# wangchou/whisper.coreml

Hardware: AMD Instinct MI355X
Metric: xRT (audio-s/s) large-v3 beam=5 @1/2/4/8 GPU; p50 per-token decode ms (higher is better)
Workload: dtype fp16; 1 GPU; large-v3 beam=5 transcribe() of one 600 s file, 30 s clip grid, condition_on_previous_text=False, temperature=0; model=large-v3, global_batch=20, seq_len=448

## Files before the change

### profiles/chain_trace.py

```python
import ctypes
import os
import sys

import numpy as np

REPO = os.path.dirname(os.path.dirname(os.path.abspath(__file__)))
sys.path[:0] = [os.path.join(REPO, "whisper.coreml_amd"), REPO]
import whisper
from whisper import synthetic as S
from whisper.decoding import DecodingTask

W = int(sys.argv[1]) if len(sys.argv) > 1 else 20
REPS = int(sys.argv[2]) if len(sys.argv) > 2 else 10
ADVANCE = int(sys.argv[3]) if len(sys.argv) > 3 else 0
model_name = os.environ.get("CT_MODEL", "large-v3")
dims = S.MODEL_DIMS[model_name]
m = whisper.Whisper(whisper.ModelDimensions(**dims), model_name, device=0, dtype="fp16", max_windows=W, max_group=5)
m.load_state_dict(S.synthetic_state_dict(dims, 0))
m.ctx.log_mel(S.synthetic_audio(30.0 * W, seed=1000), dims["n_mels"], padding=whisper.audio.N_SAMPLES)
m.ctx.encode([3000 * i for i in range(W)], [3000] * W)
task = DecodingTask(m, whisper.DecodingOptions(language="en", beam_size=5))
lib = m.ctx.lib
UNITS = ["proj", "kernels", "gemm", "decode"]
for u in UNITS:
    getattr(lib, f"wh_tune_ct_trace_{u}").argtypes = [ctypes.c_void_p]
    getattr(lib, f"wh_tune_ct_trace_{u}").restype = ctypes.c_int
    getattr(lib, f"wh_tune_ct_clear_{u}").restype = ctypes.c_int
SLOT_UNIT = {0: "proj", 1: "proj", 2: "proj", 3: "proj", 4: "kernels", 5: "kernels", 6: "kernels", 7: "kernels",
             8: "gemm", 9: "decode", 10: "decode", 11: "decode"}
ORDER = [(0, "qkv k_proj", ("X staged", "MFMA done")), (6, "self-attn (+qkv reduce)", None),
         (7, "cross-attn k_xattn_seg", None), (1, "cross-out k_proj", ("X staged", "MFMA done")),
         (2, "fc1 k_proj", ("X staged", "MFMA done")), (5, "reduce+GELU", None),
         (3, "fc2 k_proj", ("X staged", "MFMA done")), (4, "resid+LN (final)", ("loads landed", None)),
         (8, "vocab k_vocab_2p / k_vocab1", ("epilogue start", "half 1 staged")), (9, "selection k_logit_part", ("row combine", "window merge")),
         (10, "  merge_window (in it)", ("staged", "ranked")),
         (11, "  selection slices (marks)", ("loads", "top-k"))]

m.ctx.decode_begin(task.wh_opts(), [task.initial_tokens] * W, [task.sot_index] * W)
m.ctx.time_stage(0, 2 + ADVANCE)
rows = {s: [] for s, _, _ in ORDER}
steps = []
for rep in range(REPS):
    for u in UNITS:
        assert getattr(lib, f"wh_tune_ct_clear_{u}")() == 0
    steps.append(m.ctx.time_stage(0, 1))
    tr = {}
    for u in UNITS:
        buf = np.zeros((12, 2048, 4), dtype=np.uint64)
        assert getattr(lib, f"wh_tune_ct_trace_{u}")(buf.ctypes.data) == 0
        tr[u] = buf.astype(np.int64)
    base = None
    for slot, name, phases in ORDER:
        t = tr[SLOT_UNIT[slot]][slot]
        t = t[t[:, 0] > 0]
        if len(t) == 0:
            continue
        if base is None:
            base = t[:, 0].min()
        rel = (t - base) * 0.01
        ends = rel[:, 3][t[:, 3] > 0]
        rows[slot].append(dict(n=len(t), s0=rel[:, 0].min(), s1=rel[:, 0].max(),
                               p1=np.median(rel[:, 1][t[:, 1] > 0]) if (t[:, 1] > 0).any() else np.nan,
                               p2=np.median(rel[:, 2][t[:, 2] > 0]) if (t[:, 2] > 0).any() else np.nan,
                               e_med=np.median(ends) if len(ends) else np.nan, e1=ends.max() if len(ends) else np.nan,
                               p1max=rel[:, 1][t[:, 1] > 0].max() if (t[:, 1] > 0).any() else np.nan,
                               p2max=rel[:, 2][t[:, 2] > 0].max() if (t[:, 2] > 0).any() else np.nan))
print(f"{model_name} fp16, {W} windows x beam 5 ({5 * W} rows), after {2 + ADVANCE} steps: "
      f"step graph {np.median(steps):.3f} ms "
      f"(median of {REPS}); times in us from layer 31's qkv first workgroup start, medians over {REPS} steps")
print(f"{'launch':28s} {'WGs':>5s} {'gap':>6s} {'start0':>7s} {'startN':>7s} {'phase1':>7s} {'phase2':>7s} "
      f"{'end med':>7s} {'end max':>7s} {'span':>6s}")
prev_end = None
for slot, name, phases in ORDER:
    if not rows[slot]:
        continue
    agg = {k: float(np.nanmedian([r[k] for r in rows[slot]])) for k in rows[slot][0]}
    gap = agg["s0"] - prev_end if prev_end is not None else float("nan")
    print(f"{name:28s} {int(agg['n']):5d} {gap:6.2f} {agg['s0']:7.2f} {agg['s1']:7.2f} {agg['p1']:7.2f} "
          f"{agg['p2']:7.2f} {agg['e_med']:7.2f} {agg['e1']:7.2f} {agg['e1'] - agg['s0']:6.2f}"
          f"   (phase maxima {agg['p1max']:.2f} / {agg['p2max']:.2f})")
    prev_end = agg["e1"]
```

### whisper.coreml_amd/csrc/wh_kernels.hip

```cpp
#include "wh_kernels.h"

#include <cstdio>
#include <type_traits>
#include <cstdlib>

namespace wh {

template <typename T>
__global__ __launch_bounds__(256) void k_layernorm(const float* __restrict__ x, T* __restrict__ y, const float* __restrict__ gamma,
                                                   const float* __restrict__ beta, int rows, int n, float eps,
                                                   const int* __restrict__ rows_in) {
  const int row = blockIdx.x * 4 + (threadIdx.x >> 6);
  const int lane = threadIdx.x & 63;
  if (row >= rows) return;
  const int src = rows_in ? rows_in[row] : row;
  const float* xr = x + (int64_t)src * n;
  constexpr int MAXV = 8;
  float4_t v[MAXV];
  const int nv = n >> 2;
#pragma unroll
  for (int i = 0; i < MAXV; ++i) {
    const int c = lane + 64 * i;
    if (c < nv) v[i] = load4f(xr + 4 * c);
  }
// ... 400 lines not shown
      CT_END(CT_SELF_ATTN);
      return;
    }
  }
  if constexpr (sizeof(T) == 2) {
    int sv[8];
#pragma unroll
    for (int i = 0; i < 8; ++i) sv[i] = an[min(lane + 64 * i, ctx - 1)];
    qs[lane] = to_f32(q_lane);
#pragma unroll
    for (int i = 0; i < 8; ++i) {
      const int pp = lane + 64 * i;
      if (pp <= pos) slot_of[pp] = (pp == pos ? sl : sv[i]) * slotB;
    }
    asm volatile("s_waitcnt lgkmcnt(0)" ::: "memory");
    const int kg = lane >> 3, dc = (lane & 7) * 8;
    float m = -INFINITY, lsum = 0.f, o[8];
#pragma unroll
    for (int e = 0; e < 8; ++e) o[e] = 0.f;
    for (int p0 = 0; p0 <= pos; p0 += 128) {
      const int pa = min(p0 + lane, pos), pb = min(p0 + 64 + lane, pos);
      const int ra = baseB + slot_of[pa] + pa * ROWB, rb = baseB + slot_of[pb] + pb * ROWB;
      Frag<T> ka[8], kb[8], vf[16];
#pragma unroll
      for (int c = 0; c < 8; ++c) frag_load_buf(ka[c], rk, ra + 8 * c * TB);
#pragma unroll
      for (int c = 0; c < 8; ++c) frag_load_buf(kb[c], rk, rb + 8 * c * TB);
#pragma unroll
      for (int u = 0; u < 16; ++u) {
        const int pc = min(p0 + kg + 8 * u, pos);
        frag_load_buf(vf[u], rv, baseB + slot_of[pc] + pc * ROWB + dc * TB);
      }
      __builtin_amdgcn_sched_barrier(0);
      float sa = 0.f, sb = 0.f;
#pragma unroll
      for (int c = 0; c < 8; ++c) {
        const float4_t q0 = *reinterpret_cast<const float4_t*>(&qs[8 * c]);
        const float4_t q1 = *reinterpret_cast<const float4_t*>(&qs[8 * c + 4]);
#pragma unroll
        for (int e = 0; e < 8; ++e) {
          const float qe = e < 4 ? q0[e] : q1[e - 4];
          sa += qe * to_f32(ka[c].v[e]);
          sb += qe * to_f32(kb[c].v[e]);
        }
      }
      const bool va = p0 + lane <= pos, vb = p0 + 64 + lane <= pos;
      const float mp = wave_max(fmaxf(va ? sa : -INFINITY, vb ? sb : -INFINITY));
      const float mn = fmaxf(m, mp), scale = __expf(m - mn);
      m = mn;
      const float ea = va ? __expf(sa - m) : 0.f, eb = vb ? __expf(sb - m) : 0.f;
      lsum = lsum * scale + wave_sum(ea + eb);
      sc[lane] = ea;
      sc[64 + lane] = eb;
      asm volatile("s_waitcnt lgkmcnt(0)" ::: "memory");
#pragma unroll
      for (int e = 0; e < 8; ++e) o[e] *= scale;
#pragma unroll
      for (int u = 0; u < 16; ++u) {
        const float pw = sc[kg + 8 * u];
#pragma unroll
        for (int e = 0; e < 8; ++e) o[e] += pw * to_f32(vf[u].v[e]);
      }
    }
#pragma unroll
    for (int e = 0; e < 8; ++e) {
      o[e] = xor8_sum(o[e]);
      o[e] = xor16_sum(o[e]);
      o[e] = xor32_sum(o[e]);
    }
    if (kg == 0) {
      const float inv = 1.f / lsum;
      T* op = out + (int64_t)row * ldo + h * 64 + dc;
      store4(op, o[0] * inv, o[1] * inv, o[2] * inv, o[3] * inv);
      store4(op + 4, o[4] * inv, o[5] * inv, o[6] * inv, o[7] * inv);
    }
    CT_END(CT_SELF_ATTN);
    return;
  }
  qs[lane] = to_f32(q_lane);
  asm volatile("s_waitcnt lgkmcnt(0)" ::: "memory");
  unpack_q();
  float mx = -INFINITY;
  for (int p = lane; p <= pos; p += 64) {
    const int slot = ((p == pos) ? sl : an[p]) * slotB;
    slot_of[p] = slot;
    const int kr = baseB + slot + p * ROWB;
    float s = 0.f;
#pragma unroll
    for (int c = 0; c < 64; c += 8) {
      Frag<T> f;
      frag_load_buf(f, rk, kr + c * TB);
#pragma unroll
      for (int e = 0; e < 8; ++e) s += qv[c + e] * to_f32(f.v[e]);
    }
    sc[p] = s;
    mx = fmaxf(mx, s);
  }
  mx = wave_max(mx);
  float sum = 0.f;
  for (int p = lane; p <= pos; p += 64) {
    const float e = __expf(sc[p] - mx);
    sc[p] = e;
    sum += e;
  }
  sum = wave_sum(sum);
  __syncthreads();
  const int kg = lane >> 3, dc = (lane & 7) * 8;
  float o[8];
#pragma unroll
  for (int e = 0; e < 8; ++e) o[e] = 0.f;
  int p = kg;
  for (; p + 24 <= pos; p += 32) {
    Frag<T> f[4];
#pragma unroll
    for (int u = 0; u < 4; ++u) frag_load_buf(f[u], rv, baseB + slot_of[p + 8 * u] + (p + 8 * u) * ROWB + dc * TB);
#pragma unroll
    for (int u = 0; u < 4; ++u) {
      const float pw = sc[p + 8 * u];
#pragma unroll
      for (int e = 0; e < 8; ++e) o[e] += pw * to_f32(f[u].v[e]);
    }
  }
  for (; p <= pos; p += 8) {
    Frag<T> f;
    frag_load_buf(f, rv, baseB + slot_of[p] + p * ROWB + dc * TB);
    const float pw = sc[p];
#pragma unroll
    for (int e = 0; e < 8; ++e) o[e] += pw * to_f32(f.v[e]);
  }
#pragma unroll
  for (int e = 0; e < 8; ++e) {
    o[e] = xor8_sum(o[e]);
    o[e] = xor16_sum(o[e]);
    o[e] = xor32_sum(o[e]);
  }
  if (kg == 0) {
    const float inv = 1.f / sum;
    T* op = out + (int64_t)row * ldo + h * 64 + dc;
    store4(op, o[0] * inv, o[1] * inv, o[2] * inv, o[3] * inv);
    store4(op + 4, o[4] * inv, o[5] * inv, o[6] * inv, o[7] * inv);
  }
  CT_END(CT_SELF_ATTN);
}

template <typename T>
void launch_self_attn(const T* q, int ldq, const T* kc, const T* vc, const int* rw, const int* rs, const int* rp,
                      const int* anc, int anc_beams, int nbeam, int H, int ctx, T* out, int ldo, int rows,
                      hipStream_t st) {
  if (rows <= 0) return;
  k_self_attn<T><<<dim3(rows, H), 64, 0, st>>>(q, ldq, kc, vc, rw, rs, rp, anc, anc_beams, nbeam, H, ctx, out, ldo,
                                               self_attn_kco_min()), wh_launched("k_self_attn");
}

template <typename T, typename S = float>
__global__ __launch_bounds__(64) __attribute__((amdgpu_waves_per_eu(1, 2))) void k_self_attn_qkv(const S* __restrict__ part, int nsplit, int64_t part_stride,
                                                      const float* __restrict__ bqkv, int ns, T* __restrict__ kc,
                                                      T* __restrict__ vc, const int* __restrict__ row_win,
                                                      const int* __restrict__ row_slot, const int* __restrict__ row_pos,
                                                      const int* __restrict__ anc, int anc_beams, int nbeam, int H,
                                                      int ctx, T* __restrict__ out, int ldo, int kco_min = 0) {
  __shared__ float sc[512];
  __shared__ int slot_of[512];
  __shared__ float qs[64], vs[64];
  const int lane = threadIdx.x, G = anc_beams;
  CT_MARK(CT_SELF_ATTN, 0);
  const int L = xcd_remap(blockIdx.x, gridDim.x), sl = L % G, wh = L / G, h = wh % H, w = wh / H, row = w * G + sl;
  const int* an = anc + ((int64_t)w * anc_beams + sl) * ctx;
  const int64_t head_stride = (int64_t)ctx * 64;
  const int64_t wbase = (int64_t)w * nbeam;
  auto kv_off = [&](int slot, int p) -> int64_t { return ((wbase + slot) * H + h) * head_stride + (int64_t)p * 64; };
  constexpr int TB = (int)sizeof(T), ROWB = 64 * TB;
  const int slotB = H * ctx * ROWB, baseB = ((int)wbase * H + h) * ctx * ROWB;
  const auto rk = wt_rsrc(kc), rv = wt_rsrc(vc);
  const int pos = row_pos[row];
  int sv[8];
#pragma unroll
  for (int i = 0; i < 8; ++i) sv[i] = an[min(lane + 64 * i, ctx - 1)];
  float qd, kd, vd;
  {
    constexpr bool H16 = sizeof(S) == 2;
    const S* pr = part + (int64_t)row * 3 * ns + h * 64 + lane;
    qd = bqkv[h * 64 + lane];
    kd = bqkv[ns + h * 64 + lane];
    vd = bqkv[2 * ns + h * 64 + lane];
    S a0[16], a1[16], a2[16];
#pragma unroll
    for (int z = 0; z < 16; ++z)
      if (H16 || z < nsplit) {
        const int64_t zo = (int64_t)(H16 ? min(z, nsplit - 1) : z) * part_stride;
        a0[z] = pr[zo];
        a1[z] = pr[zo + ns];
        a2[z] = pr[zo + 2 * ns];
      }
    if constexpr (H16) {
      asm volatile("" ::"s"(pos));
#pragma unroll
      for (int z = 0; z < 16; ++z) asm volatile("" ::"v"(a0[z]), "v"(a1[z]), "v"(a2[z]));
    }
    auto f32 = [](S r) -> float { return (float)r; };
#pragma unroll
    for (int z = 0; z < 16; ++z)
      if (z < nsplit) {
        qd += f32(a0[z]);
        kd += f32(a1[z]);
        vd += f32(a2[z]);
      }
  }
  for (int i = 0; i < 8; ++i)
    if (lane + 64 * i < pos) slot_of[lane + 64 * i] = sv[i] * slotB;
  const int plast = max(pos - 1, 0);
  const T qT = from_f32<T>(qd), kT = from_f32<T>(kd), vT = from_f32<T>(vd);
  kc[kv_off(sl, pos) + lane] = kT;
  vc[kv_off(sl, pos) + lane] = vT;
  qs[lane] = to_f32(qT);
  vs[lane] = to_f32(vT);
  const float s_cur = wave_sum(to_f32(qT) * to_f32(kT));
  asm volatile("s_waitcnt lgkmcnt(0)" ::: "memory");
  if constexpr (sizeof(T) == 2) {
    const int kg = lane >> 3, dc = (lane & 7) * 8;
    float m = s_cur, lsum = 0.f, o[8];
#pragma unroll
    for (int e = 0; e < 8; ++e) o[e] = 0.f;
    float qd8[8];
#pragma unroll
    for (int e = 0; e < 8; ++e) qd8[e] = qs[dc + e];
    auto load = [&](auto kc, int p0, Frag<T>(&k)[8], Frag<T>(&v)[8]) {
      if constexpr (decltype(kc)::value) {
        int off[8];
#pragma unroll
        for (int u = 0; u < 8; ++u) {
          const int pc = min(p0 + kg + 8 * u, plast);
          off[u] = baseB + slot_of[pc] + pc * ROWB + dc * TB;
        }
#pragma unroll
        for (int u = 0; u < 8; ++u) frag_load_buf(k[u], rk, off[u]);
#pragma unroll
        for (int u = 0; u < 8; ++u) frag_load_buf(v[u], rv, off[u]);
        return;
      }
      const int pa = min(p0 + lane, plast);
      const int ra = baseB + slot_of[pa] + pa * ROWB;
#pragma unroll
      for (int c = 0; c < 8; ++c) frag_load_buf(k[c], rk, ra + 8 * c * TB);
#pragma unroll
      for (int u = 0; u < 8; ++u) {
        const int pc = min(p0 + kg + 8 * u, plast);
        frag_load_buf(v[u], rv, baseB + slot_of[pc] + pc * ROWB + dc * TB);
      }
    };
    auto pass = [&](auto kc, int p0, const Frag<T>(&k)[8], const Frag<T>(&v)[8]) {
      if constexpr (decltype(kc)::value) {
        kco_pass<T, 8>(qd8, k, v, p0 + kg, pos, m, lsum, o);
        return;
      }
      float sa = 0.f;
#pragma unroll
      for (int c = 0; c < 8; ++c) {
        const float4_t q0 = *reinterpret_cast<const float4_t*>(&qs[8 * c]);
        const float4_t q1 = *reinterpret_cast<const float4_t*>(&qs[8 * c + 4]);
#pragma unroll
        for (int e = 0; e < 8; ++e) sa += (e < 4 ? q0[e] : q1[e - 4]) * to_f32(k[c].v[e]);
      }
      const bool va = p0 + lane < pos;
      const float mp = wave_max(va ? sa : -INFINITY);
      const float mn = fmaxf(m, mp), scale = __expf(m - mn);
      m = mn;
      const float ea = va ? __expf(sa - m) : 0.f;
      lsum = lsum * scale + wave_sum(ea);
      sc[lane] = ea;
      asm volatile("s_waitcnt lgkmcnt(0)" ::: "memory");
#pragma unroll
      for (int e = 0; e < 8; ++e) o[e] *= scale;
#pragma unroll
      for (int u = 0; u < 8; ++u) {
        const float pw = sc[kg + 8 * u];
#pragma unroll
        for (int e = 0; e < 8; ++e) o[e] += pw * to_f32(v[u].v[e]);
      }
    };
    auto run = [&](auto kc) {
      Frag<T> ka[8], va[8], kb[8], vb[8];
      if (pos > 0) load(kc, 0, ka, va);
      int p0 = 0;
      for (; p0 + 64 < pos; p0 += 128) {
        load(kc, p0 + 64, kb, vb);
        pass(kc, p0, ka, va);
        if (p0 + 128 < pos) load(kc, p0 + 128, ka, va);
        pass(kc, p0 + 64, kb, vb);
      }
      if (p0 < pos) pass(kc, p0, ka, va);
    };
    if (pos > kco_min) run(std::true_type());
    else run(std::false_type());
#pragma unroll
    for (int e = 0; e < 8; ++e) {
      o[e] = xor8_sum(o[e]);
      o[e] = xor16_sum(o[e]);
      o[e] = xor32_sum(o[e]);
    }
    if (kg == 0) {
      const float e_cur = __expf(s_cur - m), inv = 1.f / (lsum + e_cur);
#pragma unroll
      for (int e = 0; e < 8; ++e) o[e] = (o[e] + e_cur * vs[dc + e]) * inv;
      T* op = out + (int64_t)row * ldo + h * 64 + dc;
      store4(op, o[0], o[1], o[2], o[3]);
      store4(op + 4, o[4], o[5], o[6], o[7]);
    }
    CT_END(CT_SELF_ATTN);
    return;
  }
  float qv[64];
#pragma unroll
  for (int c = 0; c < 64; ++c) qv[c] = qs[c];
  float mx = s_cur;
  for (int p0 = 0; p0 < pos; p0 += 128) {
    const int pa = min(p0 + lane, plast), pb = min(p0 + 64 + lane, plast);
    const int ra = baseB + slot_of[pa] + pa * ROWB, rb = baseB + slot_of[pb] + pb * ROWB;
    Frag<T> ka[8], kb[8];
#pragma unroll
    for (int c = 0; c < 8; ++c) frag_load_buf(ka[c], rk, ra + 8 * c * TB);
#pragma unroll
    for (int c = 0; c < 8; ++c) frag_load_buf(kb[c], rk, rb + 8 * c * TB);
    __builtin_amdgcn_sched_barrier(0);
    float sa = 0.f, sb = 0.f;
#pragma unroll
    for (int c = 0; c < 8; ++c)
#pragma unroll
      for (int e = 0; e < 8; ++e) {
        sa += qv[8 * c + e] * to_f32(ka[c].v[e]);
        sb += qv[8 * c + e] * to_f32(kb[c].v[e]);
      }
    if (p0 + lane < pos) {
      sc[p0 + lane] = sa;
      mx = fmaxf(mx, sa);
    }
    if (p0 + 64 + lane < pos) {
      sc[p0 + 64 + lane] = sb;
      mx = fmaxf(mx, sb);
    }
  }
  mx = wave_max(mx);
  float sum = 0.f;
  for (int p = lane; p < pos; p += 64) {
    const float e = __expf(sc[p] - mx);
    sc[p] = e;
    sum += e;
  }
  const float e_cur = __expf(s_cur - mx);
  sum = wave_sum(sum) + e_cur;
  asm volatile("s_waitcnt lgkmcnt(0)" ::: "memory");
  const int kg = lane >> 3, dc = (lane & 7) * 8;
  float o[8];
#pragma unroll
  for (int e = 0; e < 8; ++e) o[e] = 0.f;
  for (int p0 = kg; p0 < pos; p0 += 64) {
    Frag<T> f[8];
    float pw[8];
#pragma unroll
    for (int u = 0; u < 8; ++u) {
      const int pc = min(p0 + 8 * u, plast);
      frag_load_buf(f[u], rv, baseB + slot_of[pc] + pc * ROWB + dc * TB);
      pw[u] = p0 + 8 * u < pos ? sc[pc] : 0.f;
    }
    __builtin_amdgcn_sched_barrier(0);
#pragma unroll
    for (int u = 0; u < 8; ++u)
#pragma unroll
      for (int e = 0; e < 8; ++e) o[e] += pw[u] * to_f32(f[u].v[e]);
  }
#pragma unroll
  for (int e = 0; e < 8; ++e) {
    o[e] = xor8_sum(o[e]);
    o[e] = xor16_sum(o[e]);
    o[e] = xor32_sum(o[e]);
  }
  if (kg == 0) {
    const float inv = 1.f / sum;
#pragma unroll
    for (int e = 0; e < 8; ++e) o[e] = (o[e] + e_cur * vs[dc + e]) * inv;
    T* op = out + (int64_t)row * ldo + h * 64 + dc;
    store4(op, o[0], o[1], o[2], o[3]);
    store4(op + 4, o[4], o[5], o[6], o[7]);
  }
  CT_END(CT_SELF_ATTN);
}

int self_attn_kco_min() {
  static const int v = [] {
    const char* e = tune_env("WHISPER_HIP_SA_KCO_MIN");
    return e ? atoi(e) : 64;
  }();
  return v;
}
template <typename T>
int launch_self_attn_qkv(const float* part, int nsplit, int64_t part_stride, const float* bqkv, int ns, T* kc, T* vc,
                          const int* rw, const int* rs, const int* rp, const int* anc, int anc_beams, int nbeam, int H,
                          int ctx, T* out, int ldo, int rows, hipStream_t st, int slab_half) {
  if (rows <= 0) return 0;
  if (anc_beams < 1 || rows % anc_beams || nsplit > 16) return -1;
  if (slab_half) {
    if constexpr (sizeof(T) == 2) {
      k_self_attn_qkv<T, half_t><<<rows * H, 64, 0, st>>>(reinterpret_cast<const half_t*>(part), nsplit, part_stride,
                                                         bqkv, ns, kc, vc, rw, rs, rp, anc, anc_beams, nbeam, H, ctx,
                                                         out, ldo, self_attn_kco_min()), wh_launched("k_self_attn_qkv");
      return 0;
    }
    return -1;
  }
  k_self_attn_qkv<T><<<rows * H, 64, 0, st>>>(part, nsplit, part_stride, bqkv, ns, kc, vc, rw, rs, rp, anc, anc_beams,
                                             nbeam, H, ctx, out, ldo, self_attn_kco_min()), wh_launched("k_self_attn_qkv");
  return 0;
}

template <typename T, int ACT, typename S = float>
__global__ __launch_bounds__(256) void k_reduce_store(const S* __restrict__ part, int nsplit, int64_t part_stride,
                                                      const float* __restrict__ bias, T* __restrict__ out, int ldo, int M,
                                                      int N) {
  const int i = (int)(blockIdx.x * 256 + threadIdx.x) * 4;
  CT_MARK(CT_REDUCE, 0);
  if (i >= M * N) return;
  const int m = (int)((unsigned)i / (unsigned)N), n = i - m * N;
  typedef typename std::conditional<sizeof(S) == 2, half4_t, float4_t>::type R4;
  R4 pp[16];
#pragma unroll
  for (int z = 0; z < 16; ++z)
    if (z < nsplit) pp[z] = *reinterpret_cast<const R4*>(part + z * part_stride + i);
  float4_t v = bias ? load4f(bias + n) : (float4_t){0.f, 0.f, 0.f, 0.f};
#pragma unroll
  for (int z = 0; z < 16; ++z)
    if (z < nsplit) v += (float4_t){(float)pp[z][0], (float)pp[z][1], (float)pp[z][2], (float)pp[z][3]};
  if (ACT) {
#pragma unroll
    for (int j = 0; j < 4; ++j) v[j] = gelu_f(v[j]);
  }
  store4(out + (int64_t)m * ldo + n, v[0], v[1], v[2], v[3]);
  CT_END(CT_REDUCE);
}

template <typename T>
void launch_reduce_store(const float* part, int nsplit, int64_t part_stride, const float* bias, T* out, int ldo, int M,
                         int N, int gelu, hipStream_t st, int slab_half) {
  if (M <= 0) return;
  if ((int64_t)M * N >= (int64_t)1 << 31) {
    wh_set_launch_error("launch_reduce_store: M x N >= 2^31");
    return;
  }
  const int64_t tot = (int64_t)M * N / 4;
  const unsigned nb = (unsigned)((tot + 255) / 256);
  if (slab_half) {
    if constexpr (sizeof(T) == 2) {
      const half_t* ph = reinterpret_cast<const half_t*>(part);
      if (gelu) k_reduce_store<T, 1, half_t><<<nb, 256, 0, st>>>(ph, nsplit, part_stride, bias, out, ldo, M, N), wh_launched("k_reduce_store");
      else k_reduce_store<T, 0, half_t><<<nb, 256, 0, st>>>(ph, nsplit, part_stride, bias, out, ldo, M, N), wh_launched("k_reduce_store");
    } else {
      wh_set_launch_error("launch_reduce_store: fp16 slabs in an fp32 context");
    }
    return;
  }
  if (gelu) k_reduce_store<T, 1><<<nb, 256, 0, st>>>(part, nsplit, part_stride, bias, out, ldo, M, N), wh_launched("k_reduce_store");
  else k_reduce_store<T, 0><<<nb, 256, 0, st>>>(part, nsplit, part_stride, bias, out, ldo, M, N), wh_launched("k_reduce_store");
}

template <typename T, int NW, int QZ>
__global__ __launch_bounds__(64 * NW) void k_cross_attn(const T* __restrict__ q, int ldq, const T* ck,
                                                    const T* cvt, int Tk, int H, int nsplit,
                                                    const int* __restrict__ win_row0, const int* __restrict__ win_nrows,
                                                    const int* __restrict__ win_slot, int64_t win_stride,
                                                    float* __restrict__ po, float* __restrict__ pm, float* __restrict__ pl,
                                                    float* qk_out, const int* qk_map, int qk_rows, XQPart xq) {
  __shared__ float red_m[NW][16], red_l[NW][16];
  __shared__ float red_o[NW][64][17];
  constexpr bool QP = QZ > 0;
  __shared__ __attribute__((aligned(16))) T qs[QP ? 32 : 1][72];
  const int wi = blockIdx.x, h = blockIdx.y, sp = blockIdx.z;
  const int tid = threadIdx.x, lane = tid & 63, wave = tid >> 6;
  const int r = lane & 15, g = lane >> 4;
  const int row0 = win_row0[wi], nrows = win_nrows[wi];
  const int kt0 = (sp * NW + wave) * 64;
  const bool active = kt0 < Tk;
  const int qslot = qk_map ? qk_map[h] : -1;
  const T* kbase = ck + (int64_t)win_slot[wi] * win_stride + (int64_t)h * TKP * 64;
  const T* vbase = cvt + (int64_t)win_slot[wi] * win_stride + (int64_t)h * 64 * TKP;
  constexpr float LOG2E = 1.4426950408889634f;
  const int ktl = active ? kt0 : 0;
  Frag<T> kf[4][2], vf[4][2];
#pragma unroll
  for (int kt = 0; kt < 4; ++kt) {
    const T* kp = kbase + (int64_t)(ktl + kt * 16 + r) * 64 + 8 * g;
    frag_load(kf[kt][0], kp);
    frag_load(kf[kt][1], kp + 32);
  }
  float4_t qv = (float4_t){0.f, 0.f, 0.f, 0.f}, pp[QP ? QZ : 1];
  __builtin_amdgcn_sched_barrier(0);
  if constexpr (QP) {
    const int t = tid & 255, qq = min(t >> 4, nrows - 1), c = h * 64 + (t & 15) * 4;
    const float* src = xq.part + (int64_t)(row0 + qq) * ldq + c;
#pragma unroll
    for (int z = 0; z < QZ; ++z) pp[z] = load4f(src + z * xq.stride);
    qv = load4f(xq.bias + c);
  }
  __builtin_amdgcn_sched_barrier(0);
#pragma unroll
  for (int dt = 0; dt < 4; ++dt)
#pragma unroll
    for (int s = 0; s < 2; ++s) frag_load(vf[dt][s], vbase + ((int64_t)(ktl >> 6) * 64 + dt * 16 + r) * 64 + 32 * s + 8 * g);
  if constexpr (QP) {
#pragma unroll
    for (int z = 0; z < QZ; ++z) qv += pp[z];
    store4(&qs[tid >> 4][(tid & 15) * 4], qv[0], qv[1], qv[2], qv[3]);
    asm volatile("s_waitcnt lgkmcnt(0)\n\ts_barrier" ::: "memory");
  }
  for (int rt = 0; rt < nrows; rt += 16) {
    int qr = rt + r;
    const bool qvalid = qr < nrows;
    if (!qvalid) qr = nrows - 1;
    float m = -INFINITY, l = 0.f;
    float4_t acc[4];
#pragma unroll
    for (int i = 0; i < 4; ++i) acc[i] = (float4_t){0.f, 0.f, 0.f, 0.f};
    if (active) {
      Frag<T> qf[2];
      if constexpr (QP) {
        frag_load(qf[0], &qs[qr][8 * g]);
        frag_load(qf[1], &qs[qr][32 + 8 * g]);
      } else {
        const T* qp = q + (int64_t)(row0 + qr) * ldq + h * 64 + 8 * g;
        frag_load(qf[0], qp);
        frag_load(qf[1], qp + 32);
      }
      float4_t sc[4];
#pragma unroll
      for (int kt = 0; kt < 4; ++kt) {
        sc[kt] = (float4_t){0.f, 0.f, 0.f, 0.f};
        mfma_step(sc[kt], kf[kt][0], qf[0]);
        mfma_step(sc[kt], kf[kt][1], qf[1]);
      }
      float mx = -INFINITY;
#pragma unroll
      for (int kt = 0; kt < 4; ++kt)
#pragma unroll
        for (int j = 0; j < 4; ++j) {
          const int key = kt0 + kt * 16 + 4 * g + j;
          if (key >= Tk) sc[kt][j] = -INFINITY;
          else if (qslot >= 0 && qvalid) qk_out[((int64_t)qslot * qk_rows + row0 + qr) * Tk + key] = sc[kt][j];
          mx = fmaxf(mx, sc[kt][j]);
        }
      mx = xor16_max(mx);
      mx = xor32_max(mx);
      m = mx;
      Frag<T> pf[2];
      float ps = 0.f;
#pragma unroll
      for (int kt = 0; kt < 4; ++kt)
#pragma unroll
        for (int j = 0; j < 4; ++j) {
          const float p = hw_exp2((sc[kt][j] - m) * LOG2E);
          ps += p;
// ... 832 lines not shown
```

### whisper.coreml_amd/csrc/wh_runtime.hip

```cpp
#include <hip/hip_runtime.h>

#include <algorithm>
#include <chrono>
#include <cmath>
#include <cstdio>
#include <cstring>
#include <set>
#include <string>
#include <vector>

#include "whisper_hip.h"
#include "wh_align.h"
#include "wh_audio.h"
#include "wh_gemm.h"
#include "wh_host.h"
#include "wh_kernels.h"

using namespace wh;

static thread_local std::string g_release_error;

namespace {

constexpr int CTX = 448;
// ... 606 lines not shown
    g.out_f32 = part; g.ldo = N; g.ksplit = *ks;
    return gemm(X, ldx, W, nullptr, R, N, K, EPI_PARTIAL, g);
  }

  int resid(const T* X, int K, const T* W, const float* b, int R, const float* lg, const float* lb) {
    const int n = ns;
    GemmArgs g;
    if (R > 128) {
      g.out_f32 = x_d; g.ldo = n;
      TRY(gemm(X, K, W, b, R, n, K, EPI_RESID, g));
      launch_resid_ln<T>(x_d, nullptr, 0, 0, nullptr, xn_d, lg, lb, R, n, 1e-5f, st);
    } else {
      int ks = 0;
      TRY(partial(X, K, W, R, n, K, &ks));
      launch_resid_ln<T>(x_d, part, ks, (int64_t)R * n, b, xn_d, lg, lb, R, n, 1e-5f, st, slab_h);
    }
    return 0;
  }
  int proj(const T* W, const float* b, int R, int N, T* out, int gelu, bool skinny) {
    GemmArgs g;
    if (skinny) {
      int ks = 0;
      TRY(partial(xn_d, ns, W, R, N, ns, &ks));
      launch_reduce_store<T>(part, ks, (int64_t)R * N, b, out, N, R, N, gelu, st, slab_h);
    } else {
      g.out = out; g.ldo = N;
      TRY(gemm(xn_d, ns, W, b, R, N, ns, gelu ? EPI_STORE_GELU : EPI_STORE, g));
    }
    return 0;
  }

  int sa_probe_ks = 1;
  int sa_probe_half = 0;
  int dec_layers(int R, const int* rw, const int* rs, const int* rp, int ancG, int nwin, const int* wr0, const int* wnr,
                 const int* wsl, float* aqk, const int* qkmap, int qkrows, bool step = false,
                 const int* anc = nullptr) {
    const int* A = anc ? anc : S.anc;
    const int n = ns;
    const bool skinny = step && R <= 128;
    GemmArgs g;
    final_x = nullptr;
    if (step && !qkmap && p1_active(R, nwin))
      return dec_layers_p1(R, rw, rs, rp, ancG, nwin, wr0, wnr, wsl, A);
    launch_layernorm<T>(x_d, xn_d, dec[0].ln1_g, dec[0].ln1_b, R, n, 1e-5f, nullptr, st);
    for (int l = 0; l < Ld; ++l) {
      auto& e = dec[l];
      if (skinny) {
        int ks = 0;
        TRY(partial(xn_d, n, e.wqkv, R, 3 * n, n, &ks, slab16_qkv()));
        sa_probe_ks = ks;
        sa_probe_half = slab_h;
        if (launch_self_attn_qkv<T>(part, ks, (int64_t)R * 3 * n, e.bqkv, n, kc[l], vc[l], rw, rs, rp, A, ancG,
                                    Gcap, nh, CTX, att_d, n, R, st, slab_h))
          return fail(-20, "self-attention rows are not a whole number of beam groups");
      } else {
        g = GemmArgs();
        g.out = q_d; g.ldo = n; g.hs_state = n; g.hs_heads = nh;
        g.row_win = rw; g.row_slot = rs; g.row_pos = rp; g.kc = kc[l]; g.vc = vc[l]; g.kv_beams = Gcap; g.kv_ctx = CTX;
        TRY(gemm(xn_d, n, e.wqkv, e.bqkv, R, 3 * n, n, EPI_QKV_DEC, g));
        launch_self_attn<T>(q_d, n, kc[l], vc[l], rw, rs, rp, A, ancG, Gcap, nh, CTX, att_d, n, R, st);
      }
      TRY(resid(att_d, n, e.wo, e.bo, R, e.lnx_g, e.lnx_b));
      XQPart xq;
      if (skinny) xq = step_xq(ancG);
      if (skinny && xq_proj_active(ancG)) {
        xq.qx = xn_d; xq.qwf = e.wqx_f; xq.bias = e.bqx;
      } else if (skinny && xq_fused) {
        int ks = 0;
        TRY(partial(xn_d, n, e.wqx, R, n, n, &ks));
        if (cross_attn_q_slabs(ks)) {
          xq.part = part; xq.part_half = slab_h; xq.stride = (int64_t)R * n; xq.z = ks; xq.bias = e.bqx;
        } else {
          launch_reduce_store<T>(part, ks, (int64_t)R * n, e.bqx, q_d, n, R, n, 0, st, slab_h);
        }
      } else {
        TRY(proj(e.wqx, e.bqx, R, n, q_d, 0, skinny));
      }
      const T* ck = ckv + (size_t)(2 * l) * Wcap * TKP * n;
      const T* cv = ckv + (size_t)(2 * l + 1) * Wcap * TKP * n;
      launch_cross_attn<T>(q_d, n, ck, cv, 1500, nh, NSPLIT, nwin, wr0, wnr, wsl, (int64_t)TKP * n, po, pm, pl, att_d,
                           n, R, aqk, qkmap ? qkmap + l * nh : nullptr, qkrows, st, xq);
      TRY(resid(att_d, n, e.wox, e.box, R, e.ln2_g, e.ln2_b));
      TRY(proj(e.w1, e.b1, R, 4 * n, hm_d, 1, skinny));
      const bool last = l + 1 == Ld;
      TRY(resid(hm_d, 4 * n, e.w2, e.b2, R, last ? ln_g : dec[l + 1].ln1_g, last ? ln_b : dec[l + 1].ln1_b));
    }
    return 0;
  }

  static bool p1_enabled() {
    static const bool on = [] {
      const char* e = tune_env("WHISPER_HIP_P1");
      return !(e && e[0] == '0');
    }();
    return on;
  }

  int p1(GemmArgs& g, int epi, bool ln) {
    g.p1_slab = p1_slab;
    g.p1_cnt = p1_cnt;
    g.p1_slabs = P1_SLABS;
    const bool tev = proj_ev_n < (int)proj_ev.size() / 2;
    const int rc = tev ? launch_proj1<T>(g, epi, ln, st, proj_ev[2 * proj_ev_n], proj_ev[2 * proj_ev_n + 1])
                       : launch_proj1<T>(g, epi, ln, st);
    if (tev && rc == 0) ++proj_ev_n;
    return rc == 0 ? 0 : fail(-20, "k_proj1 launch failed code " + std::to_string(rc));
  }

  int layer_projections(int l, int R) {
    const int n = ns;
    auto& e = dec[l];
    if (p1_active(R, cur_nwin)) {
      GemmArgs g;
      g.W = e.wqkv; g.bias = e.bqkv; g.M = R; g.N = 3 * n; g.K = n;
      g.xf32 = x_d; g.ln_g = e.ln1_g; g.ln_b = e.ln1_b; g.ln_eps = 1e-5f;
      g.out = q_d; g.ldo = n; g.hs_state = n; g.hs_heads = nh;
      g.row_win = st_row_win; g.row_slot = st_row_slot; g.row_pos = row_pos; g.kc = kc[l]; g.vc = vc[l];
      g.kv_beams = Gcap; g.kv_ctx = CTX;
      TRY(p1(g, EPI_QKV_DEC, true));
      struct Q { const T* X; int K; const T* W; const float* b; int N; int epi; const float* lg; const float* lb; T* out; };
      const Q qs[5] = {{att_d, n, e.wo, e.bo, n, EPI_RESID, nullptr, nullptr, nullptr},
                       {nullptr, n, e.wqx, e.bqx, n, EPI_STORE, e.lnx_g, e.lnx_b, q_d},
                       {att_d, n, e.wox, e.box, n, EPI_RESID, nullptr, nullptr, nullptr},
                       {nullptr, n, e.w1, e.b1, 4 * n, EPI_STORE_GELU, e.ln2_g, e.ln2_b, hm_d},
                       {hm_d, 4 * n, e.w2, e.b2, n, EPI_RESID, nullptr, nullptr, nullptr}};
      for (const Q& q : qs) {
        g = GemmArgs();
        g.W = q.W; g.bias = q.b; g.M = R; g.N = q.N; g.K = q.K;
        if (q.lg) {
          g.xf32 = x_d; g.ln_g = q.lg; g.ln_b = q.lb; g.ln_eps = 1e-5f; g.out = q.out; g.ldo = q.N;
        } else {
          g.X = q.X; g.ldx = q.K; g.out_f32 = x_d; g.ldo = n;
        }
        TRY(p1(g, q.epi, q.lg != nullptr));
      }
      return 0;
    }
    struct P { const T* X; int K; const T* W; int N; } ps[6] = {
        {xn_d, n, e.wqkv, 3 * n}, {att_d, n, e.wo, n}, {xn_d, n, e.wqx, n},
        {att_d, n, e.wox, n},     {xn_d, n, e.w1, 4 * n}, {hm_d, 4 * n, e.w2, n}};
    for (auto& p : ps) {
      if (p.W == e.wqx && xq_proj_active(cur_G)) continue;
      int ks = 0;
      TRY(partial(p.X, p.K, p.W, R, p.N, p.K, &ks));
    }
    return 0;
  }

  bool p1_active(int R, int n_win) const { return n_win == 1 && p1_enabled() && proj1_supported(R, ns); }
  std::string step_kernels(int n_win, int group) const override {
    const bool p1 = p1_active(n_win * group, n_win), h = sizeof(T) == 2;
    return std::string("proj=") + (p1 ? "k_proj1" : "k_proj") + ",xattn=k_xattn_seg" +
           (!p1 && xq_proj_active(group) ? "<qproj>" : "") + ",self_attn=" +
           (p1 ? (h ? "k_self_attn<kco>" : "k_self_attn") : h ? "k_self_attn_qkv<pipe+kco>" : "k_self_attn_qkv") +
           ",tail=vocab+k_logit_part";
  }

  int dec_layers_p1(int R, const int* rw, const int* rs, const int* rp, int ancG, int nwin, const int* wr0,
                    const int* wnr, const int* wsl, const int* A) {
    const int n = ns;
    float* xc = x_d;
    float* xo = x2_d;
    const float* pend = nullptr;
    auto ln_in = [&](GemmArgs& g, const float* lg, const float* lb) {
      g.xf32 = xc; g.ln_g = lg; g.ln_b = lb; g.ln_eps = 1e-5f;
      if (pend) { g.res_slab = p1_slab; g.res_bias = pend; g.x_out = xo; }
    };
    auto ln_done = [&]() {
      if (pend) { std::swap(xc, xo); pend = nullptr; }
    };
    auto resid = [&](const T* X, int K, const T* W, const float* b, bool defer) -> int {
      GemmArgs g;
      g.X = X; g.ldx = K; g.W = W; g.bias = b; g.M = R; g.N = n; g.K = K; g.out_f32 = xc; g.ldo = n;
      g.p1_defer = defer;
      TRY(p1(g, EPI_RESID, false));
      if (defer) pend = b;
      return 0;
    };
    for (int l = 0; l < Ld; ++l) {
      auto& e = dec[l];
      GemmArgs g;
      g.W = e.wqkv; g.bias = e.bqkv; g.M = R; g.N = 3 * n; g.K = n;
      ln_in(g, e.ln1_g, e.ln1_b);
      g.out = q_d; g.ldo = n; g.hs_state = n; g.hs_heads = nh;
      g.row_win = rw; g.row_slot = rs; g.row_pos = rp; g.kc = kc[l]; g.vc = vc[l]; g.kv_beams = Gcap; g.kv_ctx = CTX;
      TRY(p1(g, EPI_QKV_DEC, true));
      ln_done();
      launch_self_attn<T>(q_d, n, kc[l], vc[l], rw, rs, rp, A, ancG, Gcap, nh, CTX, att_d, n, R, st);
      TRY(resid(att_d, n, e.wo, e.bo, false));
      XQPart xq = step_xq(ancG);
      g = GemmArgs();
      g.W = e.wqx; g.bias = e.bqx; g.M = R; g.N = n; g.K = n;
      ln_in(g, e.lnx_g, e.lnx_b);
      g.out = q_d; g.ldo = n;
      TRY(p1(g, EPI_STORE, true));
      ln_done();
      const T* ck = ckv + (size_t)(2 * l) * Wcap * TKP * n;
      const T* cv = ckv + (size_t)(2 * l + 1) * Wcap * TKP * n;
      launch_cross_attn<T>(q_d, n, ck, cv, 1500, nh, NSPLIT, nwin, wr0, wnr, wsl, (int64_t)TKP * n, po, pm, pl, att_d,
                           n, R, nullptr, nullptr, 0, st, xq);
      TRY(resid(att_d, n, e.wox, e.box, false));
      g = GemmArgs();
      g.W = e.w1; g.bias = e.b1; g.M = R; g.N = 4 * n; g.K = n;
      ln_in(g, e.ln2_g, e.ln2_b);
      g.out = hm_d; g.ldo = 4 * n;
      TRY(p1(g, EPI_STORE_GELU, true));
      ln_done();
      TRY(resid(hm_d, 4 * n, e.w2, e.b2, l + 1 < Ld));
    }
    final_x = xc;
    return 0;
  }

  const float* final_x = nullptr;
  int vocab(const int* rows_sel, int R, float* out) {
    GemmArgs g;
    g.out_f32 = out; g.ldo = V; g.x_rows = rows_sel;
    if (final_x && rows_sel) return fail(-20, "vocab: a row gather after the k_proj1 layers (xn_d not written)");
    if (final_x) {
      g.xf32 = final_x; g.ln_g = ln_g; g.ln_b = ln_b; g.ln_eps = 1e-5f;
    }
    return gemm(xn_d, ns, E, nullptr, R, V, ns, EPI_F32_COLS, g);
  }

  int set_opts(const wh_decode_opts* o, int n_win) {
    if (o->group < 1 || o->group > Gcap) return fail(-11, "group exceeds context max_group");
    const int mc = !o->beam ? 0
                   : o->max_candidates > 0 ? o->max_candidates
                                           : (int)std::nearbyint((double)o->group * (o->patience > 0 ? o->patience : 1.0));
    if (o->beam && (mc < 1 || mc > 16)) return fail(-11, "max_candidates out of range (1..16)");
    if (o->no_repeat_ngram < 0 || o->no_repeat_ngram > 16)
      return fail(-11, "no_repeat_ngram " + std::to_string(o->no_repeat_ngram) + " out of range (0..16)");
    if (!(o->repetition_penalty >= 0.f) || std::isinf(o->repetition_penalty))
      return fail(-11, "repetition_penalty must be finite and not negative (0 or 1: off)");
    const float pen = o->repetition_penalty == 0.f ? 1.f : o->repetition_penalty;
    const bool rep_on = o->no_repeat_ngram > 0 || pen != 1.f;
    if (rep_on || !bias_tab.empty()) {
      DecOpts q = DecOpts();
      q.V = V; q.ts_begin = o->timestamp_begin;
      if (!logit_slices(S, q, n_win))
        return fail(-11, std::string(!rep_on ? "phrase_bias" : bias_tab.empty() ? "no_repeat_ngram / repetition_penalty"
                                                                  : "no_repeat_ngram / repetition_penalty / phrase_bias") +
                             " need the sliced selection (k_logit_part): not with this vocabulary or "
                             "WHISPER_HIP_LOGIT_SPLIT=0");
    }
    if (!bias_tab.empty()) {
      for (size_t e = 0; e < bias_tab.size(); ++e)
        if (bias_tab[e].id >= o->eot) {
          const int j = (int)std::count_if(bias_tab.begin(), bias_tab.begin() + e + 1, [](const BiasRec& r) { return r.k == 0; }) - 1;
          return fail(-11, "phrase_bias: phrase " + std::to_string(j) + " names id " + std::to_string(bias_tab[e].id) +
                               ", not a text id (eot " + std::to_string(o->eot) + ")");
        }
    }
    O = DecOpts();
    O.no_repeat_ngram = o->no_repeat_ngram; O.repetition_penalty = pen;
    O.n_bias = (int)bias_tab.size();
    O.bias = O.n_bias ? bias_dev : nullptr;
    if (O.n_bias)
      HIPCHK(hipMemcpyAsync(bias_dev, bias_tab.data(), bias_tab.size() * sizeof(BiasRec), hipMemcpyHostToDevice, st));
    O.V = V; O.eot = o->eot; O.ts_begin = o->timestamp_begin; O.no_ts = o->no_timestamps;
    O.n_blank = std::min(o->n_blank, 3);
    for (int i = 0; i < O.n_blank; ++i) O.blank[i] = o->blank[i];
    O.blank[O.n_blank] = o->eot;
    O.n_blank += 1;
    O.suppress_blank = o->suppress_blank; O.timestamps = o->timestamps; O.max_initial = o->max_initial;
    O.beam = o->beam; O.sample_len = o->sample_len; O.n_ctx = CTX; O.temperature = o->temperature;
    h_seed = o->seed;
    std::vector<unsigned> mask((V + 31) / 32, 0u);
    for (int i = 0; i < o->n_suppress; ++i) {
      const int t = o->suppress[i];
      if (t >= 0 && t < V) mask[t >> 5] |= 1u << (t & 31);
    }
    HIPCHK(hipMemcpyAsync(suppress, mask.data(), mask.size() * 4, hipMemcpyHostToDevice, st));
    O.suppress = o->n_suppress > 0 ? suppress : nullptr;
    maxc = mc;
    S.G = o->group;
    S.maxc = 16;
    return 0;
  }

  int prefill(int w0, int nw, const std::vector<int>& toks, const std::vector<int>& nin, const int* sot_index,
              bool first_update_rows) {
    std::vector<int> rt, rp, rw, rs, wr0(nw), wnr(nw), wsl(nw), sel;
    for (int i = 0; i < nw; ++i) {
      wr0[i] = (int)rt.size();
      wnr[i] = nin[i];
      wsl[i] = win_slots[w0 + i];
      for (int p = 0; p < nin[i]; ++p) {
        rt.push_back(toks[(size_t)i * HCTX + p]);
        rp.push_back(p);
        rw.push_back(w0 + i);
        rs.push_back(0);
      }
      sel.push_back(wr0[i] + sot_index[w0 + i]);
      sel.push_back(wr0[i] + nin[i] - 1);
    }
    const int R = (int)rt.size();
    HIPCHK(hipMemcpyAsync(row_tok, rt.data(), R * 4, hipMemcpyHostToDevice, st));
    HIPCHK(hipMemcpyAsync(row_pos, rp.data(), R * 4, hipMemcpyHostToDevice, st));
    HIPCHK(hipMemcpyAsync(row_win, rw.data(), R * 4, hipMemcpyHostToDevice, st));
    HIPCHK(hipMemcpyAsync(row_slot, rs.data(), R * 4, hipMemcpyHostToDevice, st));
    HIPCHK(hipMemcpyAsync(win_row0, wr0.data(), nw * 4, hipMemcpyHostToDevice, st));
    HIPCHK(hipMemcpyAsync(win_nrows, wnr.data(), nw * 4, hipMemcpyHostToDevice, st));
    HIPCHK(hipMemcpyAsync(win_slot, wsl.data(), nw * 4, hipMemcpyHostToDevice, st));
    HIPCHK(hipMemcpyAsync(rows_in, sel.data(), sel.size() * 4, hipMemcpyHostToDevice, st));
    launch_embed<T>(E, Pdec, ns, row_tok, row_pos, nullptr, nullptr, 1, HCTX, CTX - 1, x_d, R, st);
    TRY(dec_layers(R, row_win, row_slot, row_pos, S.G, nw, win_row0, win_nrows, win_slot, nullptr, nullptr, 0));
// ... 846 lines not shown
```

Baseline: 759.5 audio-s/s.

## Overlap qkv split-K slab summation with first KV-cache tile loads in self-attn

In the fp16 pipelined path of the fused qkv-reduce + self-attention kernel, the first one or two K/V cache tiles are now issued before the partial-sum slabs are added up. Explicit vmcnt waits then let the slab loads retire while the KV loads are still in flight, so the reduction latency is hidden behind the attention prologue. The slab count is also templated (4/8/16) to cut register arrays and unused loads, and waves_per_eu is raised to a minimum of 2. The hand-counted vmcnt values are fragile and depend on the exact number of issued loads. The kco path is now forced whenever pos exceeds 64.

```diff
diff --git a/profiles/chain_trace.py b/profiles/chain_trace.py
--- a/profiles/chain_trace.py
+++ b/profiles/chain_trace.py
@@ -28,7 +28,7 @@
     getattr(lib, f"wh_tune_ct_clear_{u}").restype = ctypes.c_int
 SLOT_UNIT = {0: "proj", 1: "proj", 2: "proj", 3: "proj", 4: "kernels", 5: "kernels", 6: "kernels", 7: "kernels",
              8: "gemm", 9: "decode", 10: "decode", 11: "decode"}
-ORDER = [(0, "qkv k_proj", ("X staged", "MFMA done")), (6, "self-attn (+qkv reduce)", None),
+ORDER = [(0, "qkv k_proj", ("X staged", "MFMA done")), (6, "self-attn (+qkv reduce)", ("qkv summed", None)),
          (7, "cross-attn k_xattn_seg", None), (1, "cross-out k_proj", ("X staged", "MFMA done")),
          (2, "fc1 k_proj", ("X staged", "MFMA done")), (5, "reduce+GELU", None),
          (3, "fc2 k_proj", ("X staged", "MFMA done")), (4, "resid+LN (final)", ("loads landed", None)),
diff --git a/whisper.coreml_amd/csrc/wh_kernels.hip b/whisper.coreml_amd/csrc/wh_kernels.hip
--- a/whisper.coreml_amd/csrc/wh_kernels.hip
+++ b/whisper.coreml_amd/csrc/wh_kernels.hip
@@ -576,8 +576,8 @@
                                                self_attn_kco_min()), wh_launched("k_self_attn");
 }
 
-template <typename T, typename S = float>
-__global__ __launch_bounds__(64) __attribute__((amdgpu_waves_per_eu(1, 2))) void k_self_attn_qkv(const S* __restrict__ part, int nsplit, int64_t part_stride,
+template <typename T, typename S = float, int NS = 16>
+__global__ __launch_bounds__(64) __attribute__((amdgpu_waves_per_eu(2, 2))) void k_self_attn_qkv(const S* __restrict__ part, int nsplit, int64_t part_stride,
                                                       const float* __restrict__ bqkv, int ns, T* __restrict__ kc,
                                                       T* __restrict__ vc, const int* __restrict__ row_win,
                                                       const int* __restrict__ row_slot, const int* __restrict__ row_pos,
@@ -600,54 +600,57 @@
   int sv[8];
 #pragma unroll
   for (int i = 0; i < 8; ++i) sv[i] = an[min(lane + 64 * i, ctx - 1)];
-  float qd, kd, vd;
-  {
-    constexpr bool H16 = sizeof(S) == 2;
-    const S* pr = part + (int64_t)row * 3 * ns + h * 64 + lane;
-    qd = bqkv[h * 64 + lane];
-    kd = bqkv[ns + h * 64 + lane];
-    vd = bqkv[2 * ns + h * 64 + lane];
-    S a0[16], a1[16], a2[16];
-#pragma unroll
-    for (int z = 0; z < 16; ++z)
-      if (H16 || z < nsplit) {
-        const int64_t zo = (int64_t)(H16 ? min(z, nsplit - 1) : z) * part_stride;
-        a0[z] = pr[zo];
-        a1[z] = pr[zo + ns];
-        a2[z] = pr[zo + 2 * ns];
-      }
-    if constexpr (H16) {
-      asm volatile("" ::"s"(pos));
-#pragma unroll
-      for (int z = 0; z < 16; ++z) asm volatile("" ::"v"(a0[z]), "v"(a1[z]), "v"(a2[z]));
-    }
-    auto f32 = [](S r) -> float { return (float)r; };
-#pragma unroll
-    for (int z = 0; z < 16; ++z)
+  constexpr bool PIPE = sizeof(T) == 2 && sizeof(S) == 2;
+  const S* pr = part + (int64_t)row * 3 * ns + h * 64 + lane;
+  S a0[NS], a1[NS], a2[NS];
+#pragma unroll
+  for (int z = 0; z < NS; ++z)
+    if (PIPE || z < nsplit) {
+      const int64_t zo = (int64_t)(PIPE ? min(z, nsplit - 1) : z) * part_stride;
+      a0[z] = pr[zo];
+      a1[z] = pr[zo + ns];
+      a2[z] = pr[zo + 2 * ns];
+    }
+  float qd = bqkv[h * 64 + lane], kd = bqkv[ns + h * 64 + lane], vd = bqkv[2 * ns + h * 64 + lane];
+  auto sum_slabs = [&]() {
+#pragma unroll
+    for (int z = 0; z < NS; ++z)
       if (z < nsplit) {
-        qd += f32(a0[z]);
-        kd += f32(a1[z]);
-        vd += f32(a2[z]);
-      }
-  }
-  for (int i = 0; i < 8; ++i)
-    if (lane + 64 * i < pos) slot_of[lane + 64 * i] = sv[i] * slotB;
+        qd += (float)a0[z];
+        kd += (float)a1[z];
+        vd += (float)a2[z];
+      }
+  };
+  if constexpr (PIPE) {
+    __builtin_amdgcn_sched_barrier(0);
+    asm volatile("s_waitcnt vmcnt(%0)" ::"n"(3 * NS + 3) : "memory");
+#pragma unroll
+    for (int i = 0; i < 8; ++i) slot_of[lane + 64 * i] = (lane + 64 * i < pos ? sv[i] : 0) * slotB;
+    asm volatile("s_waitcnt lgkmcnt(0)" ::: "memory");
+  } else {
+    sum_slabs();
+    for (int i = 0; i < 8; ++i)
+      if (lane + 64 * i < pos) slot_of[lane + 64 * i] = sv[i] * slotB;
+  }
   const int plast = max(pos - 1, 0);
-  const T qT = from_f32<T>(qd), kT = from_f32<T>(kd), vT = from_f32<T>(vd);
-  kc[kv_off(sl, pos) + lane] = kT;
-  vc[kv_off(sl, pos) + lane] = vT;
-  qs[lane] = to_f32(qT);
-  vs[lane] = to_f32(vT);
-  const float s_cur = wave_sum(to_f32(qT) * to_f32(kT));
-  asm volatile("s_waitcnt lgkmcnt(0)" ::: "memory");
+  float s_cur = 0.f;
+  auto finish_qkv = [&]() {
+    const T qT = from_f32<T>(qd), kT = from_f32<T>(kd), vT = from_f32<T>(vd);
+    kc[kv_off(sl, pos) + lane] = kT;
+    vc[kv_off(sl, pos) + lane] = vT;
+    qs[lane] = to_f32(qT);
+    vs[lane] = to_f32(vT);
+    s_cur = wave_sum(to_f32(qT) * to_f32(kT));
+    asm volatile("s_waitcnt lgkmcnt(0)" ::: "memory");
+    CT_MARK(CT_SELF_ATTN, 1);
+  };
+  if constexpr (!PIPE) finish_qkv();
   if constexpr (sizeof(T) == 2) {
     const int kg = lane >> 3, dc = (lane & 7) * 8;
     float m = s_cur, lsum = 0.f, o[8];
 #pragma unroll
     for (int e = 0; e < 8; ++e) o[e] = 0.f;
     float qd8[8];
-#pragma unroll
-    for (int e = 0; e < 8; ++e) qd8[e] = qs[dc + e];
     auto load = [&](auto kc, int p0, Frag<T>(&k)[8], Frag<T>(&v)[8]) {
       if constexpr (decltype(kc)::value) {
         int off[8];
@@ -704,17 +707,38 @@
     };
     auto run = [&](auto kc) {
       Frag<T> ka[8], va[8], kb[8], vb[8];
-      if (pos > 0) load(kc, 0, ka, va);
+      if constexpr (PIPE) {
+        load(kc, 0, ka, va);
+        if (decltype(kc)::value && pos > 64) {
+          load(kc, 64, kb, vb);
+          __builtin_amdgcn_sched_barrier(0);
+          asm volatile("s_waitcnt vmcnt(32)" ::: "memory");
+          sum_slabs();
+          asm volatile("" : "+v"(qd), "+v"(kd), "+v"(vd));
+        } else {
+          __builtin_amdgcn_sched_barrier(0);
+          asm volatile("s_waitcnt vmcnt(16)" ::: "memory");
+          sum_slabs();
+        }
+        finish_qkv();
+        m = s_cur;
+      } else {
+        if (pos > 0) load(kc, 0, ka, va);
+      }
+#pragma unroll
+      for (int e = 0; e < 8; ++e) qd8[e] = qs[dc + e];
       int p0 = 0;
-      for (; p0 + 64 < pos; p0 += 128) {
-        load(kc, p0 + 64, kb, vb);
-        pass(kc, p0, ka, va);
-        if (p0 + 128 < pos) load(kc, p0 + 128, ka, va);
-        pass(kc, p0 + 64, kb, vb);
+      if constexpr (decltype(kc)::value) {
+        for (; p0 + 64 < pos; p0 += 128) {
+          if (!PIPE || p0 > 0) load(kc, p0 + 64, kb, vb);
+          pass(kc, p0, ka, va);
+          if (p0 + 128 < pos) load(kc, p0 + 128, ka, va);
+          pass(kc, p0 + 64, kb, vb);
+        }
       }
       if (p0 < pos) pass(kc, p0, ka, va);
     };
-    if (pos > kco_min) run(std::true_type());
+    if (pos > kco_min || pos > 64) run(std::true_type());
     else run(std::false_type());
 #pragma unroll
     for (int e = 0; e < 8; ++e) {
@@ -824,9 +848,15 @@
   if (anc_beams < 1 || rows % anc_beams || nsplit > 16) return -1;
   if (slab_half) {
     if constexpr (sizeof(T) == 2) {
-      k_self_attn_qkv<T, half_t><<<rows * H, 64, 0, st>>>(reinterpret_cast<const half_t*>(part), nsplit, part_stride,
-                                                         bqkv, ns, kc, vc, rw, rs, rp, anc, anc_beams, nbeam, H, ctx,
-                                                         out, ldo, self_attn_kco_min()), wh_launched("k_self_attn_qkv");
+      const half_t* ph = reinterpret_cast<const half_t*>(part);
+#define SA_QKV(NS_)                                                                                              \
+  k_self_attn_qkv<T, half_t, NS_><<<rows * H, 64, 0, st>>>(ph, nsplit, part_stride, bqkv, ns, kc, vc, rw, rs, rp, anc, \
+                                                           anc_beams, nbeam, H, ctx, out, ldo, self_attn_kco_min()),    \
+      wh_launched("k_self_attn_qkv")
+      if (nsplit <= 4) SA_QKV(4);
+      else if (nsplit <= 8) SA_QKV(8);
+      else SA_QKV(16);
+#undef SA_QKV
       return 0;
     }
     return -1;
diff --git a/whisper.coreml_amd/csrc/wh_runtime.hip b/whisper.coreml_amd/csrc/wh_runtime.hip
--- a/whisper.coreml_amd/csrc/wh_runtime.hip
+++ b/whisper.coreml_amd/csrc/wh_runtime.hip
@@ -782,7 +782,7 @@
     const bool p1 = p1_active(n_win * group, n_win), h = sizeof(T) == 2;
     return std::string("proj=") + (p1 ? "k_proj1" : "k_proj") + ",xattn=k_xattn_seg" +
            (!p1 && xq_proj_active(group) ? "<qproj>" : "") + ",self_attn=" +
-           (p1 ? (h ? "k_self_attn<kco>" : "k_self_attn") : h ? "k_self_attn_qkv<pipe+kco>" : "k_self_attn_qkv") +
+           (p1 ? (h ? "k_self_attn<kco>" : "k_self_attn") : h ? "k_self_attn_qkv<pipe+kco+kvahead>" : "k_self_attn_qkv") +
            ",tail=vocab+k_logit_part";
   }
 
```

After: 763.1 audio-s/s, median of 6. Within noise of the previous version (+0.5%).
